# lupoglaz/DeepLocalProteinDocking

Measured on AMD Instinct MI355X. Metric: pose correlations/sec (48ch x 64^3 pair, 6-degree SOI-sized generated rotation set), higher is better.
Workload: dtype f32

## Files before the change

### deeplocalproteindocking_amd/_lib.py

```python
import ctypes
import os

_HERE = os.path.dirname(os.path.abspath(__file__))
DEFAULT_PATH = os.path.join(_HERE, "csrc", "libdlpd.so")

_p = ctypes.c_void_p
_i = ctypes.c_int
_f = ctypes.c_float
_ll = ctypes.c_longlong
_sz = ctypes.c_size_t

SIGNATURES = {
    "dlpd_version": (_i, []),
    "dlpd_source_hash": (ctypes.c_char_p, []),
    "dlpd_debug_poison_lds": (_i, [_i]),
    "dlpd_debug_poison_selfcheck": (_i, [_p, _p]),
    "dlpd_grid_supported": (_i, [_i]),
    "dlpd_orientation_supported": (_i, [_i]),
    "dlpd_hidden_pad": (_i, [_i]),
    "dlpd_fused_hidden_pad": (_i, [_i, _i, _i]),
    "dlpd_generic_box_supported": (_i, [_i]),
    "dlpd_correlate_generic_ws_bytes": (_sz, [_i, _i]),
    "dlpd_correlate_generic": (_i, [_p, _p, _p, _i, _i, _i, _f, _p, _p]),
    "dlpd_local_ws_bytes": (_sz, [_i, _i, _i, _i]),
    "dlpd_local_max_poses": (_i, [_i, _i]),
    "dlpd_local_correlate": (_i, [_p, _p, _p, _p, _p, _p, _i, _i, _i, _i, _i, _i, _f, _ll, _ll, _p]),
    "dlpd_local_correlate_grad": (_i, [_p, _p, _p, _p, _p, _p, _p, _i, _i, _i, _i, _i, _i, _f, _ll, _ll, _p]),
    "dlpd_local_filter": (_i, [_p, _i, _p, _i, _p, _p, _i, _i, _i, _i, _p, _p, _p, _f, _i, _i, _f, _f, _p, _p, _p, _p]),
    "dlpd_rotate_trilinear": (_i, [_p, _p, _p, _i, _i, _i, _ll, _f, _p]),
    "dlpd_rotate_trilinear_grad": (_i, [_p, _p, _p, _i, _i, _i, _ll, _f, _i, _p]),
    "dlpd_zfft": (_i, [_p, _p, _p, _i, _i, _i, _ll, _i, _f, _p]),
    "dlpd_zfft_into": (_i, [_p, _p, _p, _i, _i, _i, _i, _i, _ll, _i, _f, _p]),
    "dlpd_zfft_volumes_occ": (_i, [_p, _p, _p, _i, _i, _i, _i, _i, _ll, _i, _p]),
    "dlpd_project_atoms": (_i, [_p, _p, _p, _p, _f, _f, _f, _p, _i, _i, _i, _i, _f, _i, _p]),
    "dlpd_project_atoms_ext": (_i, [_p, _p, _p, _p, _f, _f, _f, _p, _i, _i, _i, _i, _f, _i, _f, _i, _f, _f, _p]),
    "dlpd_project_atoms_cells": (_i, [_p, _p, _p, _p, _f, _f, _f, _p, _p, _i, _i, _i, _i, _f, _f, _i, _f, _f, _p]),
    "dlpd_rfft3d_padded": (_i, [_p, _p, _p, _i, _i, _f, _p]),
    "dlpd_xy_correlate": (_i, [_p, _p, _p, _i, _i, _i, _ll, _p]),
    "dlpd_receptor_packed_floats": (_ll, [_i, _i]),
    "dlpd_receptor_pack": (_i, [_p, _p, _i, _i, _p]),
    "dlpd_xy_correlate_packed": (_i, [_p, _p, _p, _i, _i, _i, _p]),
    "dlpd_quads_floats": (ctypes.c_size_t, [_i, _i]),
    "dlpd_make_quads": (_i, [_p, _p, _i, _i, _p]),
    "dlpd_zfft_quads": (_i, [_p, _p, _p, _i, _i, _i, _i, _i, _f, _i, _p]),
    "dlpd_channels_last_floats": (ctypes.c_size_t, [_i, _i]),
    "dlpd_make_channels_last": (_i, [_p, _p, _i, _i, _p]),
    "dlpd_zfft_channels_last": (_i, [_p, _p, _p, _i, _i, _i, _i, _i, _f, _p]),
    "dlpd_zfft_oriented": (_i, [_p, _p, _p, _i, _i, _i, _i, _i, _ll, _i, _f, _i, _p]),
    "dlpd_zfft_oriented_ext": (_i, [_p, _p, _p, _i, _i, _i, _i, _i, _ll, _i, _f, _i, _i, _p]),
    "dlpd_zfft_channels_last_ext": (_i, [_p, _p, _p, _i, _i, _i, _i, _i, _f, _i, _p]),
    "dlpd_zfft_channels_last_form": (_i, [_p, _p, _p, _i, _i, _i, _i, _i, _f, _i, _i, _p]),
    "dlpd_k1_form_supported": (_i, [_i, _i]),
    "dlpd_rotated_occupancy": (_i, [_p, _p, _p, _p, _i, _i, _f, _p]),
    "dlpd_zfft_channels_last_occ": (_i, [_p, _p, _p, _p, _i, _i, _i, _i, _i, _f, _i, _i, _p]),
    "dlpd_pencil_map_supported": (_i, [_i]),
    "dlpd_pencil_bits": (_i, [_p, _p, _i, _i, _p]),
    "dlpd_xy_correlate_packed_occ": (_i, [_p, _p, _p, _i, _i, _i, _p, _i, _p]),
    "dlpd_xy_correlate_oriented": (_i, [_p, _p, _p, _i, _i, _i, _ll, _i, _p]),
    "dlpd_score_rotations_oriented": (_i, [_p, _p, _p, _i, _i, _i, _i, _f, _p, _p, _p, _f, _i, _i, _f, _f,
                                           _p, _p, _p, _i, _p]),
    "dlpd_zifft_real": (_i, [_p, _p, _i, _i, _i, _i, _f, _p]),
    "dlpd_zifft_filter": (_i, [_p, _p, _i, _i, _i, _i, _p, _p, _p, _f, _i, _i, _f, _f, _p]),
    "dlpd_zifft_filter_cand": (_i, [_p, _p, _i, _i, _i, _i, _p, _p, _p, _f, _i, _i, _f, _f, _p, _i, _i, _p, _p, _p, _i, _p]),
    "dlpd_zifft_filter_form": (_i, [_p, _p, _i, _i, _i, _i, _p, _p, _p, _f, _i, _i, _f, _f, _p, _i, _i, _p, _p, _p, _i, _i, _p]),
    "dlpd_zifft_filter_aux": (_i, [_p, _p, _i, _i, _i, _i, _p, _p, _p, _f, _i, _i, _f, _f, _p, _i, _i, _p]),
    "dlpd_score_rotations": (_i, [_p, _p, _p, _i, _i, _i, _i, _f, _p, _p, _p, _f, _i, _i, _f, _f,
                                  _p, _p, _p, _p]),
    "dlpd_filter_mask": (_i, [_p, _i, _i, _p, _i, _i, _p, _f, _i, _p, _p, _p, _f, _i, _p, _i, _p]),
    "dlpd_filter_preact": (_i, [_p, _i, _i, _p, _p, _i, _p, _i, _p]),
    "dlpd_filter_volumes": (_i, [_p, _i, _ll, _i, _p, _i, _i, _i, _p, _ll, _f, _i, _p, _p, _p, _f, _i, _p, _i, _p]),
    "dlpd_zifft_preact": (_i, [_p, _p, _i, _i, _i, _p, _p, _i, _i, _f, _p]),
    "dlpd_zifft_preact_form": (_i, [_p, _p, _i, _i, _i, _p, _p, _i, _i, _f, _i, _p]),
    "dlpd_zifft_real_part": (_i, [_p, _p, _i, _i, _i, _i, _i, _f, _p]),
    "dlpd_maxpool3d_5s2": (_i, [_p, _p, _i, _i, _p]),
    "dlpd_maxpool3d_5s2_sparse": (_i, [_p, _p, _p, _p, _i, _i, _i, _i, _p]),
    "dlpd_conv3d_supported": (_i, [_i, _i, _i, _i]),
    "dlpd_conv3d_packed_floats": (ctypes.c_size_t, [_i, _i, _i]),
    "dlpd_conv3d_pack": (_i, [_p, _p, _i, _i, _i, _p]),
    "dlpd_conv3d": (_i, [_p, _p, _p, _i, _i, _i, _i, _i, _i, _p]),
    "dlpd_conv3d_strided": (_i, [_p, _p, _p, _i, _i, _i, _i, _i, _i, _i, _p]),
    "dlpd_conv3d_split_packed_bytes": (ctypes.c_size_t, [_i, _i, _i]),
    "dlpd_conv3d_split_pack": (_i, [_p, _p, _i, _i, _i, _p]),
    "dlpd_conv3d_split": (_i, [_p, _p, _p, _i, _i, _i, _i, _i, _i, _i, _p]),
    "dlpd_conv3d_tile_occupancy_bytes": (_sz, [_i, _i]),
    "dlpd_conv3d_tile_occupancy": (_i, [_p, _p, _i, _i, _i, _p]),
    "dlpd_conv3d_split_sparse": (_i, [_p, _p, _p, _p, _p, _i, _i, _i, _i, _i, _i, _i, _i, _p]),
    "dlpd_conv3d_wgrad_ws_floats": (_sz, [_i, _i, _i, _i]),
    "dlpd_conv3d_wgrad": (_i, [_p, _p, _p, _p, _i, _i, _i, _i, _i, _i, _p]),
# ... 3 lines not shown
    "dlpd_topk_merge_tau": (_i, [_p, _p, _p, _i, _i, _p, _p, _p]),
    "dlpd_topk_glist_bytes": (_sz, [_i]),
    "dlpd_topk_glist_reset": (_i, [_p, _i, _p]),
    "dlpd_topk_merge": (_i, [_p, _p, _p, _i, _i, _p, _p]),
}

ERRORS = {1: "DLPD_ERR_ARG (bad pointer/size)", 2: "DLPD_ERR_UNSUPPORTED (size not compiled)",
          3: "DLPD_ERR_LAUNCH (HIP launch error)"}


class DlpdLib:
    def __init__(self, path=None):
        path = path or os.environ.get("DLPD_LIB_PATH") or DEFAULT_PATH
        if not os.path.exists(path):
            raise RuntimeError(
                "dlpd: native library %s not found -- build it with "
                "`python -c 'import __graft_entry__ as g; g.build()'` (hipcc, gfx950). "
                "There is no CPU fallback." % path)
        self.path = path
        import torch
        self._dll = ctypes.CDLL(path)
        for name, (res, args) in SIGNATURES.items():
            fn = getattr(self._dll, name)
            fn.restype = res
            fn.argtypes = args
            setattr(self, "_" + name, fn)

    def source_hash(self):
        return self._dlpd_source_hash().decode()

    def call(self, name, *args):
        rc = getattr(self, "_" + name)(*args)
        if SIGNATURES[name][0] is _i and name not in ("dlpd_version", "dlpd_grid_supported", "dlpd_conv3d_supported", "dlpd_orientation_supported",
                                                      "dlpd_hidden_pad", "dlpd_fused_hidden_pad", "dlpd_generic_box_supported", "dlpd_debug_poison_selfcheck", "dlpd_k1_form_supported", "dlpd_pencil_map_supported", "dlpd_local_max_poses") and rc != 0:
            raise RuntimeError("dlpd: %s failed: %s" % (name, ERRORS.get(rc, rc)))
        return rc


_LIB = None


def get_lib():
    global _LIB
    if _LIB is None:
        _LIB = DlpdLib()
    return _LIB
```

### deeplocalproteindocking_amd/csrc/dlpd_corr.hip

```cpp
#include <dlpd_platform.h>
#include "dlpd_fft.h"
#include "dlpd_internal.h"
#include "dlpd_trilinear.h"
#include "dlpd_k1.h"
#include "dlpd_k3.h"

#ifndef DLPD_K1CL_PAD
#define DLPD_K1CL_PAD 13
#endif
#ifndef DLPD_K1CL_PXOR
#define DLPD_K1CL_PXOR 0
#endif
#define DLPD_K1_UNROLL 2
DLPD_D float trilinear_fetch_quads(const float4* __restrict__ q, int L, float px, float py, float pz) {
  const float fx = floorf(px), fy = floorf(py), fz = floorf(pz);
  const int ix = (int)fx, iy = (int)fy, iz = (int)fz;
  const float ax = px - fx, ay = py - fy, az = pz - fz;
  const int hi = L - 1;
  const bool x0 = (ix >= 0) & (ix <= hi), x1 = (ix + 1 >= 0) & (ix + 1 <= hi);
  const bool y0 = (iy >= 0) & (iy <= hi), y1 = (iy + 1 >= 0) & (iy + 1 <= hi);
  const bool z0 = (iz >= 0) & (iz <= hi), z1 = (iz + 1 >= 0) & (iz + 1 <= hi);
  const float wx0 = x0 ? 1.f - ax : 0.f, wx1 = x1 ? ax : 0.f;
  const float wy0 = y0 ? 1.f - ay : 0.f, wy1 = y1 ? ay : 0.f;
  const float wz0 = z0 ? 1.f - az : 0.f, wz1 = z1 ? az : 0.f;
// ... 142 lines not shown
    if (pencil_live) ps.load(S + p * RS, 1, t, tw);
    __syncthreads();
    if (pencil_live) ps.store(S + p * RS, 1, t);
    __syncthreads();
  }
  {
    FftPass<N, R2, R1, -1, T> ps;
    if (pencil_live) ps.load(S + p * RS, 1, t, tw);
    __syncthreads();
    if (pencil_live) ps.store(S + p * RS, 1, t);
    __syncthreads();
  }
  DLPD_STAMP(2);
  cplx* a = A + ((size_t)b * CT_out + c_base + c) * NZ * L * L + (size_t)x * L;
  for (int s = tid; s < NP * NZ; s += NT) {
    const int m = s % NP, k = s / NP;
    if (!pencil_live) continue;
    const cplx zk = S[m * RS + k];
    const cplx zn = S[m * RS + ((N - k) % N)];
    float4 o;
    o.x = 0.5f * (zk.x + zn.x);
    o.y = 0.5f * (zk.y - zn.y);
    o.z = 0.5f * (zk.y + zn.y);
    o.w = 0.5f * (zn.x - zk.x);
    DLPD_STORE_STREAM(reinterpret_cast<float4*>(a + (size_t)k * L * L + 2 * m), o);
  }
  DLPD_STAMP(3);
  }
  DLPD_STAMP_FLUSH(dlpd_stamps_k1, DLPD_STAMPS);
}

template <int N, bool OCC> __global__ void __launch_bounds__(K1ClCfg<N>::NP * FftPlan<N>::T)
k_rotate_zfft_cl(const float4* __restrict__ cl, const float* __restrict__ R, cplx* __restrict__ A,
                 int C, int Cq, int nb, float c0, int CT_out, int c_base, int ext, const unsigned char* __restrict__ occ,
                 int skip_empty) {
  constexpr int L = N / 2, NZ = N / 2 + 1, NP = K1ClCfg<N>::NP, CC = K1ClCfg<N>::CC, YG = K1ClCfg<N>::YG, NPR = YG / 2;
  constexpr int LPV = CC / 4, SKEW = 16 / LPV;
  static_assert(CC * NPR == NP && L % YG == 0 && (NP * FftPlan<N>::T) % 64 == 0, "whole waves of pencils per block");
  constexpr int RS = N + DLPD_K1CL_PAD;
  constexpr int T = FftPlan<N>::T, R1 = FftPlan<N>::R1, R2 = FftPlan<N>::R2;
  constexpr int NT = NP * T;
  DLPD_DYN_SHARED(cplx, S);
  cplx* tw = S + NP * RS;
  const int tid = threadIdx.x;
  const int nchunk = Cq / (CC / 4), per = (L / YG) * nchunk;
  const int groups = nb * L, gper = (groups + 7) / 8;
  const int bid = blockIdx.x, seq = bid >> 3;
  const int g = (bid & 7) * gper + seq / per;
  if (seq / per >= gper || g >= groups) return;
  const int inner = seq % per, yg = inner / nchunk, chunk = inner % nchunk;
  const int b = g / L, x = g % L;
  constexpr int NC = (L + 3) / 4, YC = YG / 4;
  static_assert(YG % 4 == 0, "a block's rows are whole cells");
  __shared__ unsigned char occ_s[OCC ? YC * NC : 1];
  __shared__ int occ_any;
  if (OCC) {
    const unsigned char* ob = occ + (((size_t)b * NC + (x >> 2)) * NC + (yg * YG >> 2)) * NC;
    if (tid == 0) occ_any = 0;
    __syncthreads();
    if (tid < YC * NC) {
      const unsigned char o = ob[tid];
      occ_s[tid] = o;
      if (o) occ_any = 1;
    }
    __syncthreads();
    if (!occ_any) {
      if (skip_empty) return;
      for (int s = tid; s < NP * NZ; s += NT) {
        const int pm = s % NP, k = s / NP;
        const int c = chunk * CC + pm / NPR, m = pm % NPR;
        if (c < C)
          DLPD_STORE_STREAM(reinterpret_cast<float4*>(A + (((size_t)b * CT_out + c_base + c) * NZ + k) * L * L + (size_t)x * L +
                                                      yg * YG + 2 * m), make_float4(0.f, 0.f, 0.f, 0.f));
      }
      return;
    }
  }
  init_twiddles<N>(tw, tid, NT);
  {
    const K1ClRot rot = k1cl_load_rotation(R + (size_t)b * 9);
    for (int task = tid; task < NPR * L * LPV; task += NT) {
      const int q = task % LPV, z = (task / LPV) % L, m = (task / LPV) / L;
      const float4* src = cl + chunk * (CC / 4) + q;
      float4 acc[2];
      if (OCC && !occ_s[((2 * m) >> 2) * NC + (z >> 2)])
        acc[0] = acc[1] = make_float4(0.f, 0.f, 0.f, 0.f);
      else
        k1cl_sample_rows(src, Cq, L, ext, c0, rot, x, yg * YG + 2 * m, z, acc);
      cplx* P = S + ((4 * q) * NPR + m) * RS + SKEW * q + z;
      P[0] = c_make(acc[0].x, acc[1].x);
      P[NPR * RS] = c_make(acc[0].y, acc[1].y);
      P[2 * NPR * RS] = c_make(acc[0].z, acc[1].z);
      P[3 * NPR * RS] = c_make(acc[0].w, acc[1].w);
    }
  }
  __syncthreads();
  const int p = (tid % NP) ^ DLPD_K1CL_PXOR, t = tid / NP;
  cplx* Sp = S + p * RS + SKEW * (p / (4 * NPR));
  {
    FftPass<N, R1, 1, -1, T, L> ps;
    ps.load(Sp, 1, t, tw);
    __syncthreads();
    ps.store(Sp, 1, t);
    __syncthreads();
  }
  {
    FftPass<N, R2, R1, -1, T> ps;
    ps.load(Sp, 1, t, tw);
    __syncthreads();
    ps.store(Sp, 1, t);
    __syncthreads();
  }
  for (int s = tid; s < NP * NZ; s += NT) {
    const int pm = s % NP, k = s / NP;
    const int c = chunk * CC + pm / NPR, m = pm % NPR;
    if (c < C) {
      const cplx* Z = S + pm * RS + SKEW * (pm / (4 * NPR));
      const cplx zk = Z[k];
      const cplx zn = Z[(N - k) % N];
      float4 o;
      o.x = 0.5f * (zk.x + zn.x);
      o.y = 0.5f * (zk.y - zn.y);
      o.z = 0.5f * (zk.y + zn.y);
      o.w = 0.5f * (zn.x - zk.x);
      cplx* a = A + (((size_t)b * CT_out + c_base + c) * NZ + k) * L * L + (size_t)x * L + yg * YG + 2 * m;
      DLPD_STORE_STREAM(reinterpret_cast<float4*>(a), o);
    }
  }
}

__global__ void __launch_bounds__(256) k_make_channels_last(const float* __restrict__ v, float4* __restrict__ cl, int C, int Cq, int L) {
  const size_t L3 = (size_t)L * L * L, total = L3 * Cq;
  for (size_t i = (size_t)blockIdx.x * blockDim.x + threadIdx.x; i < total; i += (size_t)gridDim.x * blockDim.x) {
    const int c4 = (int)(i % Cq);
    const size_t vox = i / Cq;
    float e[4];
#pragma unroll
    for (int j = 0; j < 4; j++) e[j] = (4 * c4 + j < C) ? v[(size_t)(4 * c4 + j) * L3 + vox] : 0.f;
    cl[i] = make_float4(e[0], e[1], e[2], e[3]);
  }
}

template <int N> static int launch_k1_cl(const float4* cl, const float* R, cplx* A, int C, int nb, float c0, hipStream_t st,
                                         int CT_out, int c_base, int ext = 0, const unsigned char* occ = nullptr, int skip_empty = 0) {
  constexpr int L = N / 2, RS = N + DLPD_K1CL_PAD;
  const int Cq = ((C + DLPD_K1CL_CC - 1) / DLPD_K1CL_CC) * (DLPD_K1CL_CC / 4);
  const size_t shmem = (size_t)(K1ClCfg<N>::NP * RS + N) * sizeof(cplx);
  const int per = (L / K1ClCfg<N>::YG) * (Cq / (K1ClCfg<N>::CC / 4));
  const int gper = (nb * L + 7) / 8;
  dim3 grid((unsigned)(8 * gper * per)), block(K1ClCfg<N>::NP * FftPlan<N>::T);
  const int e = (ext > 0 && ext < L) ? ext : L;
  if (occ) {
    int rc = dlpd_set_max_dyn_shared((const void*)k_rotate_zfft_cl<N, true>, shmem);
    if (rc) return rc;
    DLPD_LAUNCH((k_rotate_zfft_cl<N, true>), grid, block, shmem, st, cl, R, A, C, Cq, nb, c0, CT_out, c_base, e, occ, skip_empty);
  } else {
    int rc = dlpd_set_max_dyn_shared((const void*)k_rotate_zfft_cl<N, false>, shmem);
    if (rc) return rc;
    DLPD_LAUNCH((k_rotate_zfft_cl<N, false>), grid, block, shmem, st, cl, R, A, C, Cq, nb, c0, CT_out, c_base, e, occ, 0);
  }
  return dlpd_check_launch();
}

__global__ void __launch_bounds__(256) k_rotated_occupancy(const unsigned char* __restrict__ occ_src, const float* __restrict__ R,
                                                           unsigned char* __restrict__ occ_out, int nb, int L, float c0) {
  const int nc = (L + 3) / 4, nc3 = nc * nc * nc;
  for (int i = blockIdx.x * blockDim.x + threadIdx.x; i < nb * nc3; i += gridDim.x * blockDim.x) {
    const int b = i / nc3, cell = i % nc3, cz = cell % nc, cy = (cell / nc) % nc, cx = cell / (nc * nc);
    const float* r = R + (size_t)b * 9;
    const float hx = 0.5f * (min(4 * cx + 3, L - 1) - 4 * cx), hy = 0.5f * (min(4 * cy + 3, L - 1) - 4 * cy),
                hz = 0.5f * (min(4 * cz + 3, L - 1) - 4 * cz);
    const float dx = 4 * cx + hx - c0, dy = 4 * cy + hy - c0, dz = 4 * cz + hz - c0;
    bool any = false;
    int lo[3], hi[3];
#pragma unroll
    for (int a = 0; a < 3; a++) {
      const float s = c0 + (r[a] * dx + r[3 + a] * dy + r[6 + a] * dz);
      const float e = fabsf(r[a]) * hx + fabsf(r[3 + a]) * hy + fabsf(r[6 + a]) * hz + 1e-3f * (1.f + fabsf(s));
      lo[a] = max((int)floorf(s - e), 0) >> 2;
      hi[a] = min((int)floorf(s + e) + 1, L - 1) >> 2;
    }
    for (int sx = lo[0]; sx <= hi[0]; sx++)
      for (int sy = lo[1]; sy <= hi[1]; sy++)
        for (int sz = lo[2]; sz <= hi[2]; sz++) any |= occ_src[(sx * nc + sy) * nc + sz] != 0;
    occ_out[i] = any ? 1 : 0;
  }
}
__global__ void __launch_bounds__(256) k_pencil_bits(const unsigned char* __restrict__ occ, unsigned* __restrict__ bits, int nb, int nc) {
  const int lane = threadIdx.x & 63, i = (blockIdx.x * blockDim.x + threadIdx.x) >> 6;
  bool any = false;
  if (i < nb * nc && lane < nc) {
    const unsigned char* o = occ + ((size_t)i * nc + lane) * nc;
// ... 630 lines not shown
    return launch_k1_cl<2 * l()>(c4, R, A, C, nb, center, st, CT_out, c_base, extent);
  });
}

int dlpd_rotated_occupancy(const unsigned char* occ_src, const float* R, unsigned char* occ_out, unsigned* pencil_out, int nb,
                           int L, float center, void* stream) {
  if (!occ_src || !R || !occ_out || nb <= 0 || L <= 0 || L > 128) return DLPD_ERR_ARG;
  const int nc = (L + 3) / 4, total = nb * nc * nc * nc;
  DLPD_LAUNCH(k_rotated_occupancy, dim3((unsigned)((total + 255) / 256)), dim3(256), 0, (hipStream_t)stream, occ_src, R, occ_out,
              nb, L, center);
  if (pencil_out)
    DLPD_LAUNCH(k_pencil_bits, dim3((unsigned)((nb * nc + 3) / 4)), dim3(256), 0, (hipStream_t)stream, occ_out, pencil_out, nb, nc);
  return dlpd_check_launch();
}
int dlpd_pencil_bits(const unsigned char* occ, unsigned* pencil_out, int nb, int L, void* stream) {
  if (!occ || !pencil_out || nb <= 0 || L <= 0 || L > 128) return DLPD_ERR_ARG;
  const int nc = (L + 3) / 4;
  DLPD_LAUNCH(k_pencil_bits, dim3((unsigned)((nb * nc + 3) / 4)), dim3(256), 0, (hipStream_t)stream, occ, pencil_out, nb, nc);
  return dlpd_check_launch();
}
int dlpd_pencil_map_supported(int L) { return dlpd_k2_packed_receptor_floats(1, L) > 0 ? 1 : 0; }

int dlpd_zfft_channels_last_occ(const float* cl, const float* R, const unsigned char* occ, void* wsA, int nb, int C, int CT_out,
                                int c_base, int L, float center, int extent, int skip_empty, void* stream) {
  if (!cl || !R || !occ || !wsA || nb <= 0 || C <= 0 || c_base < 0 || c_base + C > CT_out || extent < 0 || extent > L) return DLPD_ERR_ARG;
  hipStream_t st = (hipStream_t)stream;
  cplx* A = (cplx*)wsA;
  const float4* c4 = (const float4*)cl;
  return dlpd_dispatch<DLPD_BOXES>(L, [&](auto l) {
    return launch_k1_cl<2 * l()>(c4, R, A, C, nb, center, st, CT_out, c_base, extent, occ, skip_empty);
  });
}

int dlpd_zfft_channels_last_ext(const float* cl, const float* R, void* wsA, int nb, int C, int CT_out, int c_base, int L,
                                float center, int extent, void* stream) {
  return dlpd_zfft_channels_last_form(cl, R, wsA, nb, C, CT_out, c_base, L, center, extent, 0, stream);
}

int dlpd_zfft_channels_last(const float* cl, const float* R, void* wsA, int nb, int C, int CT_out, int c_base, int L,
                            float center, void* stream) {
  return dlpd_zfft_channels_last_ext(cl, R, wsA, nb, C, CT_out, c_base, L, center, 0, stream);
}

int dlpd_zfft_into(const float* vol, const float* R, void* wsA, int nb, int CT, int CT_out, int c_base, int L,
                   long long vol_bstride, int do_rotate, float center, void* stream) {
  return dlpd_zfft_oriented(vol, R, wsA, nb, CT, CT_out, c_base, L, vol_bstride, do_rotate, center, 0, stream);
}

int dlpd_zfft(const float* vol, const float* R, void* wsA, int nb, int CT, int L, long long vol_bstride,
              int do_rotate, float center, void* stream) {
  return dlpd_zfft_into(vol, R, wsA, nb, CT, CT, 0, L, vol_bstride, do_rotate, center, stream);
}

int dlpd_rfft3d_padded(const float* vol, void* spec, void* wsA, int nvol, int L, float scale, void* stream) {
  if (!vol || !spec || !wsA || nvol <= 0) return DLPD_ERR_ARG;
  hipStream_t st = (hipStream_t)stream;
  int rc = dlpd_zfft(vol, nullptr, wsA, 1, nvol, L, 0, 0, 0.f, stream);
  if (rc) return rc;
  return dlpd_k2_forward((const cplx*)wsA, (cplx*)spec, nvol, 1, L, scale, st);
}

int dlpd_orientation_supported(int L) { return dlpd_k2_orientation_supported(L); }

int dlpd_xy_correlate_oriented(const void* wsA, const void* rec, void* wsB, int nb, int CT, int L,
                               long long rec_bstride, int transposed, void* stream) {
  if (!wsA || !rec || !wsB || nb <= 0 || CT <= 0) return DLPD_ERR_ARG;
// ... 183 lines not shown
```

### deeplocalproteindocking_amd/csrc/dlpd_k1.h

```cpp
#pragma once
#include <dlpd_platform.h>
#include "dlpd_fft.h"

#define DLPD_K1CL_CC 16
#ifndef DLPD_K1_YG160
#define DLPD_K1_YG160 8
#endif
#ifndef DLPD_K1_CC160
#define DLPD_K1_CC160 16
#endif
template <int N> struct K1ClCfg {
  static constexpr int YG = (N == 128) ? 16 : (N == 160 ? DLPD_K1_YG160 : 8), CC = (N == 160) ? DLPD_K1_CC160 : 128 / YG;
  static constexpr int NP = CC * (YG / 2);
};
struct K1ClRot { float r0, r1, r2, r3, r4, r5, r6, r7, r8; };
DLPD_D K1ClRot k1cl_load_rotation(const float* r) {
  K1ClRot o = {r[0], r[1], r[2], r[3], r[4], r[5], r[6], r[7], r[8]};
  return o;
}

DLPD_D void k1cl_sample_rows(const float4* __restrict__ src, int Cq, int L, int ext, float c0, const K1ClRot& r, int x, int yrow,
                             int z, float4 (&acc)[2]) {
  const float dx = x - c0, dz = z - c0;
  const int hi = L - 1;
#pragma unroll
      for (int u = 0; u < 2; u++) {
        const bool live = max(x, max(yrow + u, z)) < ext;
        const float dy = (yrow + u) - c0;
        const float px = c0 + (r.r0 * dx + r.r3 * dy + r.r6 * dz);
        const float py = c0 + (r.r1 * dx + r.r4 * dy + r.r7 * dz);
        const float pz = c0 + (r.r2 * dx + r.r5 * dy + r.r8 * dz);
        const float fx = floorf(px), fy = floorf(py), fz = floorf(pz);
        const int ix = (int)fx, iy = (int)fy, iz = (int)fz;
        const float ax = px - fx, ay = py - fy, az = pz - fz;
        const bool x0 = live & (ix >= 0) & (ix <= hi), x1 = live & (ix + 1 >= 0) & (ix + 1 <= hi);
        const bool y0 = (iy >= 0) & (iy <= hi), y1 = (iy + 1 >= 0) & (iy + 1 <= hi);
        const bool z0 = (iz >= 0) & (iz <= hi), z1 = (iz + 1 >= 0) & (iz + 1 <= hi);
        const float wx0 = x0 ? 1.f - ax : 0.f, wx1 = x1 ? ax : 0.f;
        const float wy0 = y0 ? 1.f - ay : 0.f, wy1 = y1 ? ay : 0.f;
        const float wz0 = z0 ? 1.f - az : 0.f, wz1 = z1 ? az : 0.f;
        const int cx0 = min(max(ix, 0), hi), cx1 = min(max(ix + 1, 0), hi);
        const int cy0 = min(max(iy, 0), hi), cy1 = min(max(iy + 1, 0), hi);
        const int cz0 = min(max(iz, 0), hi), cz1 = min(max(iz + 1, 0), hi);
        const float4 v000 = src[(size_t)((cx0 * L + cy0) * L + cz0) * Cq], v001 = src[(size_t)((cx0 * L + cy0) * L + cz1) * Cq];
        const float4 v010 = src[(size_t)((cx0 * L + cy1) * L + cz0) * Cq], v011 = src[(size_t)((cx0 * L + cy1) * L + cz1) * Cq];
// ... 24 lines not shown
```

### deeplocalproteindocking_amd/engine.py

```python
import numpy as np
import torch

from ._lib import get_lib


def _ptr(t):
    return 0 if t is None else t.data_ptr()


def _stream(device):
    if device.type == "cuda":
        return torch.cuda.current_stream(device).cuda_stream
    return 0


def key_to_float(key):
    key = np.asarray(key, dtype=np.uint32)
    neg = (key & np.uint32(0x80000000)) == 0
    bits = np.where(neg, ~key, key & np.uint32(0x7FFFFFFF)).astype(np.uint32)
    return bits.view(np.float32)


class DeviceTopList:

# ... 38 lines not shown
        score = key_to_float((hi >> np.uint64(32)).astype(np.uint32)).copy()
        negzero = ((lo >> np.uint64(31)) & np.uint64(1)).astype(bool)
        score[negzero] = np.float32(-0.0)
        rot = (hi & np.uint64(0xFFFFFFFF)).astype(np.int64)
        idx = (lo & np.uint64(0x7FFFFFFF)).astype(np.int64)
        pick = (lo >> np.uint64(32)).astype(np.int64)
        return rot, idx, score, pick

    @staticmethod
    def merge_entries(parts, K):
        rot = np.concatenate([p[0] for p in parts])
        idx = np.concatenate([p[1] for p in parts])
        score = np.concatenate([p[2] for p in parts])
        pick = np.concatenate([p[3] for p in parts])
        order = np.lexsort((pick, rot, score + np.float32(0.0)))[:K]
        return rot[order], idx[order], score[order], pick[order]

    @staticmethod
    def to_top_list(entries, N):
        rot, idx, score, _ = entries
        x, y, z = idx // (N * N), (idx // N) % N, idx % N
        return [(int(rot[i]), int(x[i]), int(y[i]), int(z[i]), float(score[i])) for i in range(len(rot))]


class _Grid:

    def __init__(self, eng, L, C, CT, center, extent, rot_scale, packed_receptor):
        lib, dev, nb, f32 = eng.lib, eng.device, eng.batch, torch.float32
        self.L, self.N, self.NZ, self.C, self.CT = L, 2 * L, L + 1, C, CT
        self.center = float(L) / 2.0 if center is None else float(center)
        self.extent, self.rot_scale = extent, float(rot_scale)
        N, NZ = self.N, self.NZ
        self.lig = torch.zeros(CT, L, L, L, dtype=f32, device=dev)
        self.ligcl = torch.empty(lib.call("dlpd_channels_last_floats", C, L), dtype=f32, device=dev) if eng.use_cl else None
        self.ligq = torch.empty(lib.call("dlpd_quads_floats", CT, L), dtype=f32, device=dev) if eng.use_quads else None
        npk = lib.call("dlpd_receptor_packed_floats", CT, L) if packed_receptor else 0
        self.recP = torch.zeros(npk, dtype=f32, device=dev) if npk else None
        self.recF = None if (eng._spectrum_is_temporary and self.recP is not None) else \
            torch.zeros(CT, NZ, N, N, 2, dtype=f32, device=dev)
        self.wsA = torch.empty(nb * CT * NZ * L * L * 2, dtype=f32, device=dev)
        self.wsB = torch.empty(nb * CT * NZ * N * N * 2, dtype=f32, device=dev)
        self.pencil_map_ok = self.recP is not None and bool(lib.call("dlpd_pencil_map_supported", L))
        self.occ_src = self.occ_rot = self.pen = self.fill = None
        self.sparse = self.pencil_map = False


class DockingEngine:

    def __init__(self, L, C, W1, b1, W2, b2, clip=5.0, threshold_clash=300.0, has_clash=True,
                 max_conf=1000, batch=8, device="cuda", lib=None, center=None, coarse_channels=0,
                 fine_unfused=None, channels_last=None, k3_form=0, coarse_center=None, extent=None,
                 orient=True, quads=True, prefilter=True, packed_receptor=True,
                 rotation_scale=1.0, coarse_rotation_scale=None, rotation_axis_order="xyz", clip_mode="output",
                 rotation_transpose=False, keep_receptor_spectrum=False, k1_form=0, sparse_k1=None):
        self.device = torch.device(device)
        if lib is None:
            if self.device.type != "cuda":
                raise RuntimeError("dlpd: the product path runs on an AMD GPU only "
                                   "(no CPU fallback); got device %s" % self.device)
            lib = get_lib()
        self.lib = lib
        if not lib.call("dlpd_grid_supported", int(L)):
            raise RuntimeError("dlpd: box size L=%d has no compiled fused pipeline" % L)
        self.L, self.N, self.C = int(L), 2 * int(L), int(C)
        self.has_clash = bool(has_clash)
        self.CT = self.C + (1 if self.has_clash else 0)
        rot_scale1 = float(rotation_scale if coarse_rotation_scale is None else coarse_rotation_scale)
        self.rot_axis_order, self.rot_transpose = rotation_axis_order, bool(rotation_transpose)
        self._rot_mapped = float(rotation_scale) != 1.0 or rot_scale1 != 1.0 or rotation_axis_order != "xyz" or self.rot_transpose
        if clip_mode not in ("output", "input", "none"):
            raise RuntimeError("dlpd: clip_mode %r" % (clip_mode,))
        self.clip_mode = clip_mode
        self.clip = clip
        self.threshold = float(threshold_clash)
        self.K = int(max_conf)
        self.batch = int(batch)
        dev = self.device
        f32 = torch.float32
        self.C1 = int(coarse_channels)
        self.k3_form = int(k3_form)
        self.k1_form = int(k1_form)
        if self.k1_form not in (0, 1, 2):
            raise RuntimeError("dlpd: k1_form %r (0 = library default, 1 = phased, 2 = role-split)" % (k1_form,))
        if self.k1_form == 2 and int(L) in (64, 80) and not lib.call("dlpd_k1_form_supported", int(L), 2):
            raise RuntimeError("dlpd: k1_form=2 (role-split K1) exists in -DDLPD_TEST_VARIANTS builds only; this library "
                               "(%s) does not hold it" % getattr(lib, "path", "?"))
        self.fine_unfused = bool(fine_unfused)
        self.set_filter(W1, b1, W2, b2)
        nb, CT, N = self.batch, self.CT, self.N
        self.V = torch.empty(nb, N, N, N, dtype=f32, device=dev)
        if channels_last is None:
            channels_last = self.C >= 8
        self.use_cl = bool(channels_last)
        self.extent = int(extent) if extent and int(extent) < int(L) else 0
        if self.extent and self.clip_mode == "input":
            raise RuntimeError("dlpd: clip_mode 'input' is not combined with embedded boxes (use a compiled box size)")
        self.orient = bool(orient) and not self.use_cl and bool(lib.call("dlpd_orientation_supported", int(L)))
        self.use_quads = bool(quads) and not self.use_cl and not self.extent
        self._spectrum_is_temporary = bool(self.use_cl and not keep_receptor_spectrum)
        self.prefilter = bool(prefilter)
        self.sparse_k1_wanted = sparse_k1
        self.window = None
        if self.extent:
            e = self.extent
            self.window = torch.tensor(list(range(0, e + 1)) + list(range(2 * int(L) - (e - 1), 2 * int(L))), dtype=torch.long, device=dev)
            w, Nn = self.window, 2 * int(L)
            self.window_flat = ((w[:, None, None] * Nn + w[None, :, None]) * Nn + w[None, None, :]).reshape(-1).contiguous()
            self.prefilter = False
        self.fine = _Grid(self, self.L, self.C, CT, center, self.extent, rotation_scale, packed_receptor)
        self.coarse = None
        if self.C1:
            L1 = self.L // 2
            if self.L % 2 or not lib.call("dlpd_grid_supported", L1):
                raise RuntimeError("dlpd: coarse box size %d has no compiled pipeline" % L1)
            self.coarse = _Grid(self, L1, self.C1, self.C1, coarse_center, self.extent // 2, rot_scale1, packed_receptor)
            self.pre = torch.empty(nb, self.HP, 2 * L1, 2 * L1, 2 * L1, dtype=f32, device=dev)
        self.grids = [g for g in (self.fine, self.coarse) if g is not None]
        if self.fine_unfused:
            self.conv = torch.empty(nb, CT, N, N, N, dtype=f32, device=dev)
        self.top = DeviceTopList(self.K, nb, dev, lib)
        self.clash_provider = None
        self._Vbuf = self._side = self._pending = None

    @property
    def _out_clip(self):
        on = self.clip is not None and self.clip_mode == "output"
        return (1 if on else 0), float(self.clip if on else 0.0)

    @property
    def _in_clip(self):
        return float(self.clip) if (self.clip is not None and self.clip_mode == "input") else None

    def _kernel_R(self, R, g):
        if not self._rot_mapped:
            return R
        from .Utils.Conventions import kernel_matrices
        return kernel_matrices(R, g.rot_scale, self.rot_axis_order, self.rot_transpose)

    def _k1_form_at(self, L):
        return self.k1_form if int(L) in (64, 80) else 0

    def switches(self):
        fine, c = self.fine, self.coarse
        return {"k1": "channels_last" if self.use_cl else "per_channel",
                "k1_slab_orientation": bool(self.orient), "k1_quad_layout": bool(self.use_quads),
                "k1_form": {0: "library default", 1: "phased", 2: "role-split"}[self.k1_form],
                "k3_form": {0: "library default (role-split where compiled)", 1: "channel-owning", 2: "role-split"}[self.k3_form],
                "k3_unfused": bool(self.fine_unfused), "topk_candidate_lists": bool(self.prefilter),
                "k2_packed_receptor": {"fine": fine.recP is not None, "coarse": bool(c and c.recP is not None)},
                "embedded_extent": self.extent or None,
                "k1_occupancy_maps": {"fine": fine.sparse, "coarse": bool(c and c.sparse),
                                      "k2_pencil_map": {"fine": fine.pencil_map, "coarse": bool(c and c.pencil_map)},
                                      "ligand_cells_occupied": {"fine": fine.fill, "coarse": c.fill if c else None}},
                "rotation": {"center": fine.center, "scale": fine.rot_scale, "axis_order": self.rot_axis_order,
                             "transpose": self.rot_transpose},
                "clip_mode": self.clip_mode}

    def set_filter(self, W1, b1, W2, b2):
        f32, dev, lib = torch.float32, self.device, self.lib
        W1 = torch.as_tensor(W1, dtype=f32).reshape(-1, self.C + self.C1)
        H = W1.shape[0]
        HP = lib.call("dlpd_fused_hidden_pad", int(H), self.L, int(self.C1 > 0))
        if HP < 0:
            raise RuntimeError("dlpd: hidden width %d has no fused filter kernel at box %d" % (H, self.L))
        if HP > 32 and (self.fine_unfused or self.k3_form == 1):
            raise RuntimeError("dlpd: hidden width %d runs on the role-split K3 only" % H)
        if getattr(self, "HP", HP) != HP:
            raise RuntimeError("dlpd: a live engine keeps its hidden width (%d), got %d" % (self.HP, HP))
        self.H, self.HP = H, HP
        W1t = torch.zeros(self.C + self.C1, HP, dtype=f32)
        W1t[:, :H] = W1.t()
        b1p = torch.zeros(HP, dtype=f32)
        b1p[:H] = torch.as_tensor(b1, dtype=f32).reshape(-1)
        W2p = torch.zeros(HP, dtype=f32)
        W2p[:H] = torch.as_tensor(W2, dtype=f32).reshape(-1)
        self.W1t, self.b1, self.W2 = W1t.to(dev), b1p.to(dev), W2p.to(dev)
        self.b2 = float(torch.as_tensor(b2).reshape(-1)[0])
# ... 19 lines not shown

    SPARSE_K1_MAX_FILL = 0.7

    def _ligand_occupancy(self):
        from . import ops
        for g in self.grids:
            g.sparse = g.pencil_map = False
        if not self.use_cl or self.sparse_k1_wanted is False:
            return

        def reach(occ):
            o = occ.to(torch.float32).reshape(1, 1, *occ.shape[-3:])
            return float(torch.nn.functional.max_pool3d(o, kernel_size=3, stride=1, padding=1).mean())
        for g in self.grids:
            g.occ_src = ops.tile_occupancy(g.lig[: g.C].unsqueeze(0), lib=self.lib)
            g.fill = float(g.occ_src.float().mean())
            g.sparse = bool(self.sparse_k1_wanted) or reach(g.occ_src) < self.SPARSE_K1_MAX_FILL
            if g.sparse and g.occ_rot is None:
                nc = (g.L + 3) // 4
                g.occ_rot = torch.empty(self.batch, nc, nc, nc, dtype=torch.uint8, device=self.device)
                g.pen = torch.empty(self.batch, nc, dtype=torch.int32, device=self.device)
            g.pencil_map = g.sparse and g.pencil_map_ok

    def set_ligand(self, lig_volumes, lig_forbidden=None, lig_coarse=None):
        L, fine, coarse = self.L, self.fine, self.coarse
        if coarse:
            coarse.lig.copy_(torch.as_tensor(lig_coarse, dtype=torch.float32).reshape(coarse.lig.shape))
        fine.lig[: self.C] = torch.as_tensor(lig_volumes, dtype=torch.float32).reshape(self.C, L, L, L).to(self.device)
        if self.has_clash:
            fine.lig[self.C] = torch.as_tensor(lig_forbidden, dtype=torch.float32).reshape(L, L, L).to(self.device)
        st = _stream(self.device)
        for g in self.grids:
            if self.use_cl:
                self.lib.call("dlpd_make_channels_last", _ptr(g.lig), _ptr(g.ligcl), g.C, g.L, st)
            elif self.use_quads:
                self.lib.call("dlpd_make_quads", _ptr(g.lig), _ptr(g.ligq), g.CT, g.L, st)
        self._ligand_occupancy()

    @staticmethod
    def prefers_quads(R):
        R = np.asarray(R)
        inplane = np.maximum(np.abs(R[:, 0, 2]), np.abs(R[:, 1, 2]))
        return inplane > np.abs(R[:, 2, 2])

    @staticmethod
    def prefers_transposed(R):
        R = np.asarray(R)
        return np.abs(R[:, 0, 2]) > np.abs(R[:, 1, 2])

    def _k1(self, g, R, nb, tr, quads, nch, st):
        call, L, c0 = self.lib.call, g.L, g.center
        if self.use_cl:
            if g.sparse and self._k1_form_at(L) in (0, 1):
                pen = g.pen if g.pencil_map else None
                call("dlpd_rotated_occupancy", _ptr(g.occ_src), _ptr(R), _ptr(g.occ_rot), _ptr(pen), nb, L, c0, st)
                call("dlpd_zfft_channels_last_occ", _ptr(g.ligcl), _ptr(R), _ptr(g.occ_rot), _ptr(g.wsA), nb, g.C, g.CT, 0, L,
                     c0, g.extent, int(g.pencil_map), st)
                return pen
            call("dlpd_zfft_channels_last_form", _ptr(g.ligcl), _ptr(R), _ptr(g.wsA), nb, g.C, g.CT, 0, L, c0, g.extent,
                 self._k1_form_at(L), st)
        elif quads:
            call("dlpd_zfft_quads", _ptr(g.ligq), _ptr(R), _ptr(g.wsA), nb, nch, g.CT, 0, L, c0, tr, st)
        else:
            call("dlpd_zfft_oriented_ext", _ptr(g.lig), _ptr(R), _ptr(g.wsA), nb, nch, g.CT, 0, L, 0, 1, c0, tr, g.extent, st)
        return None

    def _k1_volumes(self, g, vols, occ, st):
        call, nb, L = self.lib.call, vols.shape[0], g.L
        if occ is None:
            call("dlpd_zfft_into", _ptr(vols), 0, _ptr(g.wsA), nb, g.C, g.CT, 0, L, g.C * L ** 3, 0, 0.0, st)
            return None
        pen = None
        if g.pencil_map_ok:
            pen = torch.empty(nb, (L + 3) // 4, dtype=torch.int32, device=self.device)
            call("dlpd_pencil_bits", _ptr(occ), _ptr(pen), nb, L, st)
        call("dlpd_zfft_volumes_occ", _ptr(vols), _ptr(occ), _ptr(g.wsA), nb, g.C, g.CT, 0, L, g.C * L ** 3, int(pen is not None), st)
        return pen

    def _k2(self, g, nb, tr, pen, st):
        if pen is not None:
            assert g.recP is not None and not tr
            self.lib.call("dlpd_xy_correlate_packed_occ", _ptr(g.wsA), _ptr(g.recP), _ptr(g.wsB), nb, g.CT, g.L, _ptr(pen), g.C, st)
        elif g.recP is not None and not tr:
            self.lib.call("dlpd_xy_correlate_packed", _ptr(g.wsA), _ptr(g.recP), _ptr(g.wsB), nb, g.CT, g.L, st)
        else:
            if g.recF is None:
                raise RuntimeError("dlpd: this engine holds only the packed receptor spectrum; a transposed launch needs "
                                   "keep_receptor_spectrum=True")
            self.lib.call("dlpd_xy_correlate_oriented", _ptr(g.wsA), _ptr(g.recF), _ptr(g.wsB), nb, g.CT, g.L, 0, tr, st)

    def score_batch(self, R, mark=None, out=None, volumes=None, transposed=False, quads=False, cset=None, occupancy=None):
# ... 227 lines not shown
```

### include/dlpd.h

```cpp
#ifndef DLPD_H
#define DLPD_H
#include <stddef.h>
#ifdef __cplusplus
extern "C" {
#endif

#define DLPD_OK 0
#define DLPD_ERR_ARG 1
#define DLPD_ERR_UNSUPPORTED 2
#define DLPD_ERR_LAUNCH 3

int dlpd_version(void);
const char* dlpd_source_hash(void);
int dlpd_grid_supported(int L);
int dlpd_orientation_supported(int L);
int dlpd_hidden_pad(int H);
int dlpd_fused_hidden_pad(int H, int L, int two_res);

int dlpd_rotate_trilinear(const float* vol, const float* R, float* out, int B, int C, int L,
                          long long vol_bstride, float center, void* stream);
int dlpd_rotate_trilinear_grad(const float* gout, const float* R, float* gvol, int B, int C, int L, long long gvol_bstride,
                               float center, int accumulate, void* stream);

int dlpd_zfft(const float* vol, const float* R, void* wsA, int nb, int CT, int L, long long vol_bstride,
// ... 4 lines not shown
int dlpd_zfft_volumes_occ(const float* vol, const unsigned char* occ, void* wsA, int nb, int CT, int CT_out, int c_base, int L,
                          long long vol_bstride, int skip_empty, void* stream);

int dlpd_zfft_oriented(const float* vol, const float* R, void* wsA, int nb, int CT, int CT_out, int c_base, int L,
                       long long vol_bstride, int do_rotate, float center, int transposed, void* stream);
int dlpd_xy_correlate_oriented(const void* wsA, const void* rec, void* wsB, int nb, int CT, int L,
                               long long rec_bstride, int transposed, void* stream);

size_t dlpd_quads_floats(int nvol, int L);
int dlpd_make_quads(const float* vol, float* quads, int nvol, int L, void* stream);
int dlpd_zfft_quads(const float* quads, const float* R, void* wsA, int nb, int CT, int CT_out, int c_base, int L,
                    float center, int transposed, void* stream);

size_t dlpd_channels_last_floats(int C, int L);
int dlpd_make_channels_last(const float* vol, float* cl, int C, int L, void* stream);
int dlpd_zfft_channels_last(const float* cl, const float* R, void* wsA, int nb, int C, int CT_out, int c_base, int L,
                            float center, void* stream);

int dlpd_zfft_oriented_ext(const float* vol, const float* R, void* wsA, int nb, int CT, int CT_out, int c_base, int L,
                           long long vol_bstride, int do_rotate, float center, int transposed, int extent, void* stream);
int dlpd_zfft_channels_last_ext(const float* cl, const float* R, void* wsA, int nb, int C, int CT_out, int c_base, int L,
                                float center, int extent, void* stream);
int dlpd_k1_form_supported(int L, int form);
int dlpd_zfft_channels_last_form(const float* cl, const float* R, void* wsA, int nb, int C, int CT_out, int c_base, int L,
                                 float center, int extent, int form, void* stream);
int dlpd_rotated_occupancy(const unsigned char* occ_src, const float* R, unsigned char* occ_out, unsigned* pencil_out, int nb,
                           int L, float center, void* stream);
int dlpd_pencil_bits(const unsigned char* occ, unsigned* pencil_out, int nb, int L, void* stream);
int dlpd_zfft_channels_last_occ(const float* cl, const float* R, const unsigned char* occ, void* wsA, int nb, int C, int CT_out,
                                int c_base, int L, float center, int extent, int skip_empty, void* stream);
int dlpd_pencil_map_supported(int L);
int dlpd_xy_correlate_packed_occ(const void* wsA, const void* rec_packed, void* wsB, int nb, int CT, int L,
                                 const unsigned* pencil_map, int nmasked, void* stream);

int dlpd_project_atoms(const float* coords, const int* num_atoms_of_type, const int* offsets, const float* R,
                       float shift_x, float shift_y, float shift_z, float* out, int B, int stride_atoms,
                       int ntypes, int L, float resolution, int sum_types, void* stream);
int dlpd_project_atoms_ext(const float* coords, const int* num_atoms_of_type, const int* offsets, const float* R,
                           float shift_x, float shift_y, float shift_z, float* out, int B, int stride_atoms,
                           int ntypes, int L, float resolution, int sum_types, float sigma, int window,
                           float voxel_offset, float norm, void* stream);
int dlpd_project_atoms_cells(const float* coords, const int* num_atoms_of_type, const int* offsets, const float* R,
                             float shift_x, float shift_y, float shift_z, float* out, unsigned char* occ, int B, int stride_atoms,
                             int ntypes, int L, float resolution, float sigma, int window, float voxel_offset, float norm,
                             void* stream);

int dlpd_rfft3d_padded(const float* vol, void* spec, void* wsA, int nvol, int L, float scale, void* stream);

int dlpd_xy_correlate(const void* wsA, const void* rec, void* wsB, int nb, int CT, int L,
                      long long rec_bstride, void* stream);

long long dlpd_receptor_packed_floats(int CT, int L);
int dlpd_receptor_pack(const void* rec, void* packed, int CT, int L, void* stream);
int dlpd_xy_correlate_packed(const void* wsA, const void* rec_packed, void* wsB, int nb, int CT, int L, void* stream);

int dlpd_generic_box_supported(int L);
size_t dlpd_correlate_generic_ws_bytes(int nvol, int L);
int dlpd_correlate_generic(const float* v1, const float* v2, float* out, int nvol, int L, int has_clip, float clip,
                           void* ws, void* stream);

size_t dlpd_local_ws_bytes(int P, int C, int L, int r);
int dlpd_local_max_poses(int C, int L);
int dlpd_local_correlate(const float* rec, const float* lig, const float* R, const int* T, float* corr, void* ws, int P, int C,
                         int L, int r, int scale, int coarse_mode, float center, long long rec_pstride, long long lig_pstride,
                         void* stream);
int dlpd_local_correlate_grad(const float* rec, const float* lig, const float* R, const int* T, const float* gcorr, float* grec,
// ... 101 lines not shown
```

Baseline: 6.770 billion.

## Add chunk-major channel layout for rotate+z-FFT ligand source

Adds a new ligand source layout in which each group of CC channels is stored contiguously across the whole volume (chunk-major), instead of interleaving all channels per voxel. The rotate+z-FFT kernel takes separate voxel and chunk strides, so each block's trilinear gathers touch a compact slab rather than striding over all channels. It is enabled by default for box sizes listed in DLPD_K1_CHUNK_MAJOR_BOXES (default 64, which matches the workload). This aims to improve cache locality of the scattered rotation samples, at the cost of a separate packing kernel and extra code paths.

```diff
diff --git a/deeplocalproteindocking_amd/_lib.py b/deeplocalproteindocking_amd/_lib.py
--- a/deeplocalproteindocking_amd/_lib.py
+++ b/deeplocalproteindocking_amd/_lib.py
@@ -54,6 +54,10 @@
     "dlpd_rotated_occupancy": (_i, [_p, _p, _p, _p, _i, _i, _f, _p]),
     "dlpd_zfft_channels_last_occ": (_i, [_p, _p, _p, _p, _i, _i, _i, _i, _i, _f, _i, _i, _p]),
     "dlpd_pencil_map_supported": (_i, [_i]),
+    "dlpd_channel_chunks_floats": (ctypes.c_size_t, [_i, _i]),
+    "dlpd_channel_chunks_default": (_i, [_i]),
+    "dlpd_make_channel_chunks": (_i, [_p, _p, _i, _i, _p]),
+    "dlpd_zfft_channel_chunks": (_i, [_p, _p, _p, _p, _i, _i, _i, _i, _i, _f, _i, _i, _p]),
     "dlpd_pencil_bits": (_i, [_p, _p, _i, _i, _p]),
     "dlpd_xy_correlate_packed_occ": (_i, [_p, _p, _p, _i, _i, _i, _p, _i, _p]),
     "dlpd_xy_correlate_oriented": (_i, [_p, _p, _p, _i, _i, _i, _ll, _i, _p]),
@@ -123,7 +127,7 @@
     def call(self, name, *args):
         rc = getattr(self, "_" + name)(*args)
         if SIGNATURES[name][0] is _i and name not in ("dlpd_version", "dlpd_grid_supported", "dlpd_conv3d_supported", "dlpd_orientation_supported",
-                                                      "dlpd_hidden_pad", "dlpd_fused_hidden_pad", "dlpd_generic_box_supported", "dlpd_debug_poison_selfcheck", "dlpd_k1_form_supported", "dlpd_pencil_map_supported", "dlpd_local_max_poses") and rc != 0:
+                                                      "dlpd_hidden_pad", "dlpd_fused_hidden_pad", "dlpd_generic_box_supported", "dlpd_debug_poison_selfcheck", "dlpd_k1_form_supported", "dlpd_pencil_map_supported", "dlpd_channel_chunks_default", "dlpd_local_max_poses") and rc != 0:
             raise RuntimeError("dlpd: %s failed: %s" % (name, ERRORS.get(rc, rc)))
         return rc
 
diff --git a/deeplocalproteindocking_amd/csrc/dlpd_corr.hip b/deeplocalproteindocking_amd/csrc/dlpd_corr.hip
--- a/deeplocalproteindocking_amd/csrc/dlpd_corr.hip
+++ b/deeplocalproteindocking_amd/csrc/dlpd_corr.hip
@@ -198,8 +198,8 @@
 
 template <int N, bool OCC> __global__ void __launch_bounds__(K1ClCfg<N>::NP * FftPlan<N>::T)
 k_rotate_zfft_cl(const float4* __restrict__ cl, const float* __restrict__ R, cplx* __restrict__ A,
-                 int C, int Cq, int nb, float c0, int CT_out, int c_base, int ext, const unsigned char* __restrict__ occ,
-                 int skip_empty) {
+                 int C, int nchunk, int vstride, int cstride, int nb, float c0, int CT_out, int c_base, int ext,
+                 const unsigned char* __restrict__ occ, int skip_empty) {
   constexpr int L = N / 2, NZ = N / 2 + 1, NP = K1ClCfg<N>::NP, CC = K1ClCfg<N>::CC, YG = K1ClCfg<N>::YG, NPR = YG / 2;
   constexpr int LPV = CC / 4, SKEW = 16 / LPV;
   static_assert(CC * NPR == NP && L % YG == 0 && (NP * FftPlan<N>::T) % 64 == 0, "whole waves of pencils per block");
@@ -209,12 +209,16 @@
   DLPD_DYN_SHARED(cplx, S);
   cplx* tw = S + NP * RS;
   const int tid = threadIdx.x;
-  const int nchunk = Cq / (CC / 4), per = (L / YG) * nchunk;
+  const int per = (L / YG) * nchunk;
   const int groups = nb * L, gper = (groups + 7) / 8;
   const int bid = blockIdx.x, seq = bid >> 3;
   const int g = (bid & 7) * gper + seq / per;
   if (seq / per >= gper || g >= groups) return;
+#ifdef DLPD_K1_CHUNK_OUTER
+  const int inner = seq % per, chunk = inner / (L / YG), yg = inner % (L / YG);
+#else
   const int inner = seq % per, yg = inner / nchunk, chunk = inner % nchunk;
+#endif
   const int b = g / L, x = g % L;
   constexpr int NC = (L + 3) / 4, YC = YG / 4;
   static_assert(YG % 4 == 0, "a block's rows are whole cells");
@@ -247,12 +251,12 @@
     const K1ClRot rot = k1cl_load_rotation(R + (size_t)b * 9);
     for (int task = tid; task < NPR * L * LPV; task += NT) {
       const int q = task % LPV, z = (task / LPV) % L, m = (task / LPV) / L;
-      const float4* src = cl + chunk * (CC / 4) + q;
+      const float4* src = cl + (size_t)chunk * cstride + q;
       float4 acc[2];
       if (OCC && !occ_s[((2 * m) >> 2) * NC + (z >> 2)])
         acc[0] = acc[1] = make_float4(0.f, 0.f, 0.f, 0.f);
       else
-        k1cl_sample_rows(src, Cq, L, ext, c0, rot, x, yg * YG + 2 * m, z, acc);
+        k1cl_sample_rows(src, vstride, L, ext, c0, rot, x, yg * YG + 2 * m, z, acc);
       cplx* P = S + ((4 * q) * NPR + m) * RS + SKEW * q + z;
       P[0] = c_make(acc[0].x, acc[1].x);
       P[NPR * RS] = c_make(acc[0].y, acc[1].y);
@@ -307,23 +311,42 @@
   }
 }
 
+__global__ void __launch_bounds__(256) k_make_channel_chunks(const float* __restrict__ v, float4* __restrict__ out, int C, int CCq,
+                                                             int nchunk, int L) {
+  const size_t L3 = (size_t)L * L * L, total = L3 * CCq * nchunk;
+  for (size_t i = (size_t)blockIdx.x * blockDim.x + threadIdx.x; i < total; i += (size_t)gridDim.x * blockDim.x) {
+    const int q = (int)(i % CCq);
+    const size_t vox = (i / CCq) % L3;
+    const int c0 = 4 * ((int)(i / (CCq * L3)) * CCq + q);
+    float e[4];
+#pragma unroll
+    for (int j = 0; j < 4; j++) e[j] = (c0 + j < C) ? v[(size_t)(c0 + j) * L3 + vox] : 0.f;
+    out[i] = make_float4(e[0], e[1], e[2], e[3]);
+  }
+}
+
 template <int N> static int launch_k1_cl(const float4* cl, const float* R, cplx* A, int C, int nb, float c0, hipStream_t st,
-                                         int CT_out, int c_base, int ext = 0, const unsigned char* occ = nullptr, int skip_empty = 0) {
-  constexpr int L = N / 2, RS = N + DLPD_K1CL_PAD;
+                                         int CT_out, int c_base, int ext = 0, const unsigned char* occ = nullptr, int skip_empty = 0,
+                                         bool chunk_major = false) {
+  constexpr int L = N / 2, RS = N + DLPD_K1CL_PAD, CCq = K1ClCfg<N>::CC / 4;
   const int Cq = ((C + DLPD_K1CL_CC - 1) / DLPD_K1CL_CC) * (DLPD_K1CL_CC / 4);
+  const int nchunk = chunk_major ? (C + 4 * CCq - 1) / (4 * CCq) : Cq / CCq;
+  const int vstride = chunk_major ? CCq : Cq, cstride = chunk_major ? L * L * L * CCq : CCq;
   const size_t shmem = (size_t)(K1ClCfg<N>::NP * RS + N) * sizeof(cplx);
-  const int per = (L / K1ClCfg<N>::YG) * (Cq / (K1ClCfg<N>::CC / 4));
+  const int per = (L / K1ClCfg<N>::YG) * nchunk;
   const int gper = (nb * L + 7) / 8;
   dim3 grid((unsigned)(8 * gper * per)), block(K1ClCfg<N>::NP * FftPlan<N>::T);
   const int e = (ext > 0 && ext < L) ? ext : L;
   if (occ) {
     int rc = dlpd_set_max_dyn_shared((const void*)k_rotate_zfft_cl<N, true>, shmem);
     if (rc) return rc;
-    DLPD_LAUNCH((k_rotate_zfft_cl<N, true>), grid, block, shmem, st, cl, R, A, C, Cq, nb, c0, CT_out, c_base, e, occ, skip_empty);
+    DLPD_LAUNCH((k_rotate_zfft_cl<N, true>), grid, block, shmem, st, cl, R, A, C, nchunk, vstride, cstride, nb, c0, CT_out,
+                c_base, e, occ, skip_empty);
   } else {
     int rc = dlpd_set_max_dyn_shared((const void*)k_rotate_zfft_cl<N, false>, shmem);
     if (rc) return rc;
-    DLPD_LAUNCH((k_rotate_zfft_cl<N, false>), grid, block, shmem, st, cl, R, A, C, Cq, nb, c0, CT_out, c_base, e, occ, 0);
+    DLPD_LAUNCH((k_rotate_zfft_cl<N, false>), grid, block, shmem, st, cl, R, A, C, nchunk, vstride, cstride, nb, c0, CT_out,
+                c_base, e, occ, 0);
   }
   return dlpd_check_launch();
 }
@@ -1020,6 +1043,42 @@
   });
 }
 
+#ifndef DLPD_K1_CHUNK_MAJOR_BOXES
+#define DLPD_K1_CHUNK_MAJOR_BOXES 64
+#endif
+static int k1_chunk_channels(int L) {
+  int cc = 0;
+  dlpd_dispatch<DLPD_BOXES>(L, [&](auto l) { cc = K1ClCfg<2 * l()>::CC; return DLPD_OK; });
+  return cc;
+}
+int dlpd_channel_chunks_default(int L) { return dlpd_listed<DLPD_K1_CHUNK_MAJOR_BOXES>(L) ? 1 : 0; }
+
+size_t dlpd_channel_chunks_floats(int C, int L) {
+  const int cc = k1_chunk_channels(L);
+  return (cc && C > 0) ? (size_t)L * L * L * (size_t)(((C + cc - 1) / cc) * cc) : 0;
+}
+
+int dlpd_make_channel_chunks(const float* vol, float* buf, int C, int L, void* stream) {
+  if (!vol || !buf || C <= 0 || L <= 0) return DLPD_ERR_ARG;
+  const int cc = k1_chunk_channels(L);
+  if (!cc) return DLPD_ERR_UNSUPPORTED;
+  const int nchunk = (C + cc - 1) / cc;
+  const size_t total = (size_t)L * L * L * (cc / 4) * nchunk;
+  size_t nblk = (total + 255) / 256;
+  if (nblk > 65536) nblk = 65536;
+  DLPD_LAUNCH(k_make_channel_chunks, dim3((unsigned)nblk), dim3(256), 0, (hipStream_t)stream, vol, (float4*)buf, C, cc / 4, nchunk, L);
+  return dlpd_check_launch();
+}
+
+int dlpd_zfft_channel_chunks(const float* buf, const float* R, const unsigned char* occ, void* wsA, int nb, int C, int CT_out,
+                             int c_base, int L, float center, int extent, int skip_empty, void* stream) {
+  if (!buf || !R || !wsA || nb <= 0 || C <= 0 || c_base < 0 || c_base + C > CT_out || extent < 0 || extent > L) return DLPD_ERR_ARG;
+  return dlpd_dispatch<DLPD_BOXES>(L, [&](auto l) {
+    return launch_k1_cl<2 * l()>((const float4*)buf, R, (cplx*)wsA, C, nb, center, (hipStream_t)stream, CT_out, c_base, extent, occ,
+                                 occ ? skip_empty : 0, true);
+  });
+}
+
 int dlpd_zfft_channels_last_ext(const float* cl, const float* R, void* wsA, int nb, int C, int CT_out, int c_base, int L,
                                 float center, int extent, void* stream) {
   return dlpd_zfft_channels_last_form(cl, R, wsA, nb, C, CT_out, c_base, L, center, extent, 0, stream);
diff --git a/deeplocalproteindocking_amd/csrc/dlpd_k1.h b/deeplocalproteindocking_amd/csrc/dlpd_k1.h
--- a/deeplocalproteindocking_amd/csrc/dlpd_k1.h
+++ b/deeplocalproteindocking_amd/csrc/dlpd_k1.h
@@ -9,8 +9,11 @@
 #ifndef DLPD_K1_CC160
 #define DLPD_K1_CC160 16
 #endif
+#ifndef DLPD_K1_YG128
+#define DLPD_K1_YG128 16
+#endif
 template <int N> struct K1ClCfg {
-  static constexpr int YG = (N == 128) ? 16 : (N == 160 ? DLPD_K1_YG160 : 8), CC = (N == 160) ? DLPD_K1_CC160 : 128 / YG;
+  static constexpr int YG = (N == 128) ? DLPD_K1_YG128 : (N == 160 ? DLPD_K1_YG160 : 8), CC = (N == 160) ? DLPD_K1_CC160 : 128 / YG;
   static constexpr int NP = CC * (YG / 2);
 };
 struct K1ClRot { float r0, r1, r2, r3, r4, r5, r6, r7, r8; };
diff --git a/deeplocalproteindocking_amd/engine.py b/deeplocalproteindocking_amd/engine.py
--- a/deeplocalproteindocking_amd/engine.py
+++ b/deeplocalproteindocking_amd/engine.py
@@ -94,7 +94,10 @@
         self.extent, self.rot_scale = extent, float(rot_scale)
         N, NZ = self.N, self.NZ
         self.lig = torch.zeros(CT, L, L, L, dtype=f32, device=dev)
-        self.ligcl = torch.empty(lib.call("dlpd_channels_last_floats", C, L), dtype=f32, device=dev) if eng.use_cl else None
+        want = eng.k1_chunk_major if eng.k1_chunk_major is not None else bool(lib.call("dlpd_channel_chunks_default", L))
+        self.chunk_major = bool(eng.use_cl and want and eng._k1_form_at(L) in (0, 1))
+        self.ligcl = torch.empty(lib.call("dlpd_channel_chunks_floats" if self.chunk_major else "dlpd_channels_last_floats", C, L),
+                                 dtype=f32, device=dev) if eng.use_cl else None
         self.ligq = torch.empty(lib.call("dlpd_quads_floats", CT, L), dtype=f32, device=dev) if eng.use_quads else None
         npk = lib.call("dlpd_receptor_packed_floats", CT, L) if packed_receptor else 0
         self.recP = torch.zeros(npk, dtype=f32, device=dev) if npk else None
@@ -114,7 +117,8 @@
                  fine_unfused=None, channels_last=None, k3_form=0, coarse_center=None, extent=None,
                  orient=True, quads=True, prefilter=True, packed_receptor=True,
                  rotation_scale=1.0, coarse_rotation_scale=None, rotation_axis_order="xyz", clip_mode="output",
-                 rotation_transpose=False, keep_receptor_spectrum=False, k1_form=0, sparse_k1=None):
+                 rotation_transpose=False, keep_receptor_spectrum=False, k1_form=0, sparse_k1=None,
+                 k1_chunk_major=None):
         self.device = torch.device(device)
         if lib is None:
             if self.device.type != "cuda":
@@ -154,6 +158,7 @@
         if channels_last is None:
             channels_last = self.C >= 8
         self.use_cl = bool(channels_last)
+        self.k1_chunk_major = None if k1_chunk_major is None else bool(k1_chunk_major)
         self.extent = int(extent) if extent and int(extent) < int(L) else 0
         if self.extent and self.clip_mode == "input":
             raise RuntimeError("dlpd: clip_mode 'input' is not combined with embedded boxes (use a compiled box size)")
@@ -204,7 +209,9 @@
 
     def switches(self):
         fine, c = self.fine, self.coarse
+        layout = lambda g: None if not (g and self.use_cl) else ("chunk_major" if g.chunk_major else "channels_last")
         return {"k1": "channels_last" if self.use_cl else "per_channel",
+                "k1_source_layout": {"fine": layout(fine), "coarse": layout(c)},
                 "k1_slab_orientation": bool(self.orient), "k1_quad_layout": bool(self.use_quads),
                 "k1_form": {0: "library default", 1: "phased", 2: "role-split"}[self.k1_form],
                 "k3_form": {0: "library default (role-split where compiled)", 1: "channel-owning", 2: "role-split"}[self.k3_form],
@@ -290,7 +297,8 @@
         st = _stream(self.device)
         for g in self.grids:
             if self.use_cl:
-                self.lib.call("dlpd_make_channels_last", _ptr(g.lig), _ptr(g.ligcl), g.C, g.L, st)
+                self.lib.call("dlpd_make_channel_chunks" if g.chunk_major else "dlpd_make_channels_last", _ptr(g.lig), _ptr(g.ligcl),
+                              g.C, g.L, st)
             elif self.use_quads:
                 self.lib.call("dlpd_make_quads", _ptr(g.lig), _ptr(g.ligq), g.CT, g.L, st)
         self._ligand_occupancy()
@@ -312,9 +320,12 @@
             if g.sparse and self._k1_form_at(L) in (0, 1):
                 pen = g.pen if g.pencil_map else None
                 call("dlpd_rotated_occupancy", _ptr(g.occ_src), _ptr(R), _ptr(g.occ_rot), _ptr(pen), nb, L, c0, st)
-                call("dlpd_zfft_channels_last_occ", _ptr(g.ligcl), _ptr(R), _ptr(g.occ_rot), _ptr(g.wsA), nb, g.C, g.CT, 0, L,
-                     c0, g.extent, int(g.pencil_map), st)
+                call("dlpd_zfft_channel_chunks" if g.chunk_major else "dlpd_zfft_channels_last_occ", _ptr(g.ligcl), _ptr(R),
+                     _ptr(g.occ_rot), _ptr(g.wsA), nb, g.C, g.CT, 0, L, c0, g.extent, int(g.pencil_map), st)
                 return pen
+            if g.chunk_major:
+                call("dlpd_zfft_channel_chunks", _ptr(g.ligcl), _ptr(R), 0, _ptr(g.wsA), nb, g.C, g.CT, 0, L, c0, g.extent, 0, st)
+                return None
             call("dlpd_zfft_channels_last_form", _ptr(g.ligcl), _ptr(R), _ptr(g.wsA), nb, g.C, g.CT, 0, L, c0, g.extent,
                  self._k1_form_at(L), st)
         elif quads:
diff --git a/include/dlpd.h b/include/dlpd.h
--- a/include/dlpd.h
+++ b/include/dlpd.h
@@ -60,6 +60,11 @@
 int dlpd_pencil_map_supported(int L);
 int dlpd_xy_correlate_packed_occ(const void* wsA, const void* rec_packed, void* wsB, int nb, int CT, int L,
                                  const unsigned* pencil_map, int nmasked, void* stream);
+size_t dlpd_channel_chunks_floats(int C, int L);
+int dlpd_channel_chunks_default(int L);
+int dlpd_make_channel_chunks(const float* vol, float* buf, int C, int L, void* stream);
+int dlpd_zfft_channel_chunks(const float* buf, const float* R, const unsigned char* occ, void* wsA, int nb, int C, int CT_out,
+                             int c_base, int L, float center, int extent, int skip_empty, void* stream);
 
 int dlpd_project_atoms(const float* coords, const int* num_atoms_of_type, const int* offsets, const float* R,
                        float shift_x, float shift_y, float shift_z, float* out, int B, int stride_atoms,
```

After: 6.950 billion (median of 6 runs). 1.03x the previous value.
